# AechPro/rlgym-ppo

Measured on AMD Instinct MI355X. Metric: ppo_update_samples_per_sec, higher is better.
Workload: dtype f32; 1 GPU; configs[1]: 4096 agents x 128 steps = 524,288-sample buffer, obs 107 f32, 90 discrete actions, 256x3 policy + critic; batch 524,288, minibatch 65,536

## Files before the change

### rlgym_ppo_amd/csrc/api.hip

```cpp
#include "build_id.h"
#include <math.h>
#include <stdarg.h>
#include <string.h>

#include "common.hpp"

namespace rlppo {

static thread_local char g_err[512] = "";

void set_error(const char *fmt, ...) {
    va_list ap;
    va_start(ap, fmt);
    vsnprintf(g_err, sizeof(g_err), fmt, ap);
    va_end(ap);
}

static int64_t padded_width(int64_t d) {
    const int64_t p16 = round_up(d, 16), p64 = round_up(d, 64);
    return (p64 - p16) * 10 >= p64 ? p16 : p64;
}
static int64_t padded_out(int64_t d) {
    if (d <= 32) return 32;
    if (d <= 64) return 64;
// ... 39 lines not shown

struct X3Layout {
    int64_t fwd[RLPPO_MAX_LAYERS], dx[RLPPO_MAX_LAYERS], total;
};
static void x3_layout(const NetLayout &net, X3Layout *o) {
    int64_t off = 0;
    const int last = net.n_layers - 1;
    for (int l = 0; l < net.n_layers; ++l) {
        const LayerLayout &L = net.L[l];
        o->fwd[l] = o->dx[l] = -1;
        if (l >= 1 && l < last && nt_split_ok(L.pout, L.pin)) {
            o->fwd[l] = off;
            off += (int64_t)3 * L.pout * L.pin;
        }
        if (l >= 1 && !(l == last && gemv_head_ok(L.out, L.pin)) && nt_split_ok(L.pin, L.pout)) {
            o->dx[l] = off;
            off += (int64_t)3 * L.pin * L.pout;
        }
    }
    o->total = off;
}

static int g_fold_vhead = 1;

struct RowSource {
    const float *x;
    int64_t ld;
    const unsigned *rowtab = nullptr;
    int64_t src_rows = 0;
};

static int forward(hipStream_t st, const NetLayout &net, const float *packed, const RowSource &in, int64_t n, int out_tanh,
                   float *const *acts, int bf16_operands = 0, unsigned long long *const *bits = nullptr, bool *have_bits = nullptr,
                   bool *head_folded = nullptr, const unsigned short *x3 = nullptr, bool head_prezeroed = false) {
    X3Layout xl;
    if (x3) x3_layout(net, &xl);
    if (have_bits)
        for (int l = 0; l < net.n_layers; ++l) have_bits[l] = false;
    const float *x = in.x;
    int64_t ldx = in.ld;
    const int hl = net.n_layers - 1;
    bool fold = head_folded && g_fold_vhead && hl >= 1 && !out_tanh && !bf16_operands && bits && bits[hl - 1] &&
                gemv_head_ok(net.L[hl].out, net.L[hl].pin) && net.L[hl - 1].pout / 128 <= 2;
    if (x3 && hl >= 1 && xl.fwd[hl - 1] >= 0) fold = false;
    if (head_folded) *head_folded = false;
    for (int l = 0; l < net.n_layers; ++l) {
        const LayerLayout &L = net.L[l];
        const bool last = l == net.n_layers - 1;
        const int epi = last ? (out_tanh ? EPI_BIAS_TANH : EPI_BIAS) : EPI_BIAS_RELU;
        int rc;
        if (last && head_folded && *head_folded) break;
        if (last && !out_tanh && gemv_head_ok(L.out, L.pin))
            rc = launch_gemv_fwd(st, x, ldx, packed + L.off_w, packed + L.off_b, acts[l], L.pout, n, L.pin, L.pout);
        else {
            rc = -1;
            if (!last && bits && bits[l] && x3 && xl.fwd[l] >= 0) {
                rc = launch_gemm_nt_split(st, x, ldx, x3 + xl.fwd[l], packed + L.off_b, acts[l], L.pout, n, L.pout, L.pin, 0, bits[l]);
                if (rc == 0) have_bits[l] = true;
            } else if (!last && bits && bits[l] && !bf16_operands) {
                NtDot dots[2];
                const bool fold_here = fold && l == hl - 1;
                if (fold_here) {
                    if (!head_prezeroed) RLPPO_HIP(hipMemsetAsync(acts[hl], 0, (size_t)n * sizeof(float), st));
                    dots[0].w = packed + net.L[hl].off_w;
                    dots[0].b = packed + net.L[hl].off_b;
                    dots[0].out = acts[hl];
                }
                rc = launch_gemm_nt_bits(st, x, ldx, packed + L.off_w, L.pin, packed + L.off_b, acts[l], L.pout, n, L.pout, L.pin,
                                         EPI_BIAS_RELU, bits[l], l == 0 ? in.rowtab : nullptr, in.src_rows, nullptr, fold_here ? dots : nullptr);
                if (rc == 0) have_bits[l] = true;
                if (fold_here) *head_folded = rc == 0;
            }
            if (l == 0 && in.rowtab && rc != 0) {
                if (rc == -1) set_error("forward: the gathered first layer needs the bitmask form");
                return rc == -1 ? RLPPO_ERR_ARG : rc;
            }
            if (rc == -1)
                rc = launch_gemm_nt(st, x, ldx, packed + L.off_w, L.pin, packed + L.off_b, nullptr, 0, acts[l], L.pout, n, L.pout,
                                    L.pin, epi, bf16_operands);
        }
        if (rc) return rc;
        x = acts[l];
        ldx = L.pout;
    }
// ... 67 lines not shown
        ldx = L.pout;
    }
    return 0;
}

static size_t forward_ws_floats(const NetLayout &net, int64_t n) { return (size_t)2 * (size_t)n * (size_t)max_pout(net); }

static int forward_pingpong(hipStream_t st, const NetLayout &net, const float *packed, const float *obs, int64_t ld_obs,
                            int64_t n, int out_tanh, void *ws, size_t ws_bytes, float *final_out, const float **out,
                            int64_t *ld_out, int bf16_operands) {
    if (ws_bytes < forward_ws_floats(net, n) * sizeof(float)) {
        set_error("forward: workspace %zu < %zu bytes", ws_bytes, forward_ws_floats(net, n) * sizeof(float));
        return RLPPO_ERR_WORKSPACE;
    }
    RLPPO_CHECK_ARG(ld_obs >= net.L[0].pin && ld_obs % 4 == 0, "forward: ld_obs=%ld must be >= %d (zero padded rows)",
                    (long)ld_obs, net.L[0].pin);
    float *b0 = reinterpret_cast<float *>(ws);
    float *b1 = b0 + (size_t)n * max_pout(net);
    float *acts[RLPPO_MAX_LAYERS];
    for (int l = 0; l < net.n_layers; ++l) acts[l] = (l & 1) ? b1 : b0;
    if (final_out) acts[net.n_layers - 1] = final_out;
    int rc = forward(st, net, packed, RowSource{obs, ld_obs}, n, out_tanh, acts, bf16_operands);
    if (rc) return rc;
    *out = acts[net.n_layers - 1];
    *ld_out = net.L[net.n_layers - 1].pout;
    return 0;
}

}

using namespace rlppo;

static int g_fused_act = 1;
static std::atomic<long long> g_cnt_fused_act{0}, g_cnt_act_chain{0}, g_cnt_paired_pass{0}, g_cnt_gather_fused_pass{0}, g_cnt_pass{0}, g_cnt_group_dw{0};
constexpr int64_t FUSED_ACT_MAX_ROWS = 8192;

struct ActCtx {
    int bf16 = 0;
    unsigned *done = nullptr;
    unsigned done_value = 0;
    unsigned *noise_ctl = nullptr;
};
static int act_ctx(const rlppo_act_opts *o, ActCtx *c, bool late_noise = false) {
    c->bf16 = get_infer_bf16();
    if (!o) return 0;
    RLPPO_CHECK_ARG(o->precision == RLPPO_PRECISION_DEFAULT || o->precision == RLPPO_PRECISION_FP32 || o->precision == RLPPO_PRECISION_BF16,
                    "act options: inference precision %d (0 = process default, 1 = fp32, 2 = bf16 operands)", o->precision);
    if (o->precision != RLPPO_PRECISION_DEFAULT) c->bf16 = o->precision == RLPPO_PRECISION_BF16;
    c->done = o->done_words;
    c->done_value = o->done_value;
    c->noise_ctl = o->noise_ctl;
    RLPPO_CHECK_ARG(!o->noise_ctl || late_noise, "act options: noise_ctl is an option of rlppo_discrete_step");
    RLPPO_CHECK_ARG(!o->noise_ctl || (o->done_words && !(o->done_value & 0x80000000u)),
                    "act options: noise_ctl needs done_words (a kernel that gives up on the noise reports it there) and done_value < 2^31");
    return 0;
}
static int act_done(hipStream_t st, const ActCtx &c, int64_t n) {
    return c.done ? launch_signal_words(st, c.done, (int)rlppo_act_done_words(n), c.done_value) : 0;
}

extern "C" {

int rlppo_abi_version(void) { return RLPPO_ABI_VERSION; }
const char *rlppo_build_id(void) { return RLPPO_BUILD_ID; }
const char *rlppo_last_error(void) { return g_err; }

int64_t rlppo_padded_width(int64_t d) { return padded_width(d); }
// ... 656 lines not shown
    hipStream_t st, side;
    DwList *defer;
};

static LossCfg loss_cfg(const rlppo_minibatch_args &a) {
    LossCfg c;
    c.clip = a.clip_range;
    c.clip_lo = (float)(1.0 - (double)a.clip_range);
    c.clip_hi = (float)(1.0 + (double)a.clip_range);
    c.ent_coef = a.ent_coef;
    c.mb_ratio = a.mb_ratio;
    c.inv_mb = 1.0f / (float)a.mb;
    c.var_m = a.var_m;
    c.var_b = a.var_b;
    c.adv_norm = a.adv_norm;
    c.vclip = a.value_clip;
    c.kl_slots = a.kl_slots;
    c.stop_word = a.stop_word;
    return c;
}

static int policy_loss(hipStream_t st, const Pass &p) {
    const rlppo_minibatch_args &a = *p.a;
    const int last = p.pol.n_layers - 1;
    const LayerLayout &L = p.pol.L[last];
    const WsPlan &w = p.w;
    if (a.head == RLPPO_HEAD_DISCRETE)
        return launch_discrete_loss(st, w.pol.act[last], L.pout, L.out, w.g_act, w.g_old, w.g_adv, p.mb, p.cfg, a.stats);
    if (a.head == RLPPO_HEAD_GAUSSIAN)
        return launch_gaussian_loss(st, w.pol.act[last], L.pout, L.out / 2, w.g_act, w.g_old, w.g_adv, p.mb, p.cfg, a.stats);
    return launch_multidiscrete_loss(st, w.pol.act[last], L.pout, w.g_act, w.g_old, w.g_adv, p.mb, p.cfg, a.stats);
}

static int gather(const Pass &p) {
    const rlppo_minibatch_args &a = *p.a;
    const WsPlan &w = p.w;
    const int width = p.pol.L[0].pin;
    float *const vout = w.val.act[p.val.n_layers - 1];
    if (p.prec == 1) {
        auto lean0 = [](const NetLayout &n) {
            return n.n_layers > 1 && nt_b16_ok(n.L[0].pout, n.L[0].pin, true) && tn_b16_ok(n.L[0].pout, n.L[0].pin);
        };
        const int rc = launch_gather_rows_round(p.st, a.states, a.ld_states, a.idx, lean0(p.pol) && lean0(p.val) ? nullptr : w.states,
                                                w.states_b, width, p.mb, p.ring_base, p.ring_cap);
        if (rc) return rc;
    } else if (!p.rows.rowtab) {
        GatherMeta gm;
        gm.actions = a.actions; gm.old_logp = a.old_logp; gm.adv = a.advantages; gm.targets = a.targets;
        gm.g_old = w.g_old; gm.g_adv = w.g_adv; gm.g_tgt = w.g_tgt; gm.g_act = w.g_act;
        gm.zero_n = vout;
        gm.act_dim = a.act_dim;
        return launch_gather_rows(p.st, a.states, a.ld_states, a.idx, w.states, width, p.mb, p.ring_base, p.ring_cap, &gm);
    }
    return launch_gather_meta(p.st, a.idx, a.actions, a.act_dim, a.old_logp, a.advantages, a.targets, w.g_act, w.g_old, w.g_adv, w.g_tgt,
                              p.mb, p.ring_base, p.ring_cap, p.rows.rowtab ? w.rowtab : nullptr, vout);
}

static int paired_pass(const Pass &p, SlotBank &bk, int slot) {
    const rlppo_minibatch_args &a = *p.a;
    const NetLayout &pol = p.pol, &val = p.val;
    const WsPlan &w = p.w;
    const int64_t mb = p.mb;
    const hipStream_t st = p.st, hs = p.side;
    const int H = pol.n_layers - 1;
    int rc;
    const LayerLayout &Lvh = val.L[H];
// ... 8 lines not shown
        alt.A = xv;
        alt.B = p.val_w + Lv.off_w;
        alt.bias = p.val_w + Lv.off_b;
        alt.C = w.val.act[l];
        alt.bits = w.val.bits[l];
        NtDot dots[2];
        const bool fold_here = fold_v && l == H - 1;
        if (fold_here) {
            dots[1].w = p.val_w + Lvh.off_w;
            dots[1].out = vout;
            dots[1].b = p.val_w + Lvh.off_b;
        }
        rc = launch_gemm_nt_bits(st, xp, ldx, p.pol_w + Lp.off_w, Lp.pin, p.pol_w + Lp.off_b, w.pol.act[l], Lp.pout, mb, Lp.pout, Lp.pin,
                                 EPI_BIAS_RELU, w.pol.bits[l], l == 0 ? p.rows.rowtab : nullptr, p.rows.src_rows, &alt,
                                 fold_here ? dots : nullptr);
        if (rc) {
            if (rc == -1) set_error("paired pass: a hidden layer does not have the bitmask form");
            return rc == -1 ? RLPPO_ERR_ARG : rc;
        }
        xp = w.pol.act[l];
        xv = w.val.act[l];
        ldx = Lp.pout;
    }
    if (hs != st) {
        rc = order_after(hs, st, bk.ev_fork[slot]);
        if (rc) return rc;
    }
    if (!fold_v) {
        rc = head_forward(hs, val, p.val_w, xv, ldx, mb, 0, vout);
        if (rc) return rc;
    }
    rc = launch_value_loss(hs, vout, ldv, w.g_tgt, w.g_adv, mb, p.cfg, a.stats);
    if (rc) return rc;
    const bool ordered = g_head_order && hs != st;
    if (!ordered) {
        rc = head_backward(hs, val, p.val_w, vout, xv, mb, w.val.dx[H - 1], a.val_grad, w.val.tn, w.val.bits[H - 1], ldv, p.defer);
        if (rc) return rc;
    }
    rc = head_forward(st, pol, p.pol_w, xp, ldx, mb, a.head == RLPPO_HEAD_GAUSSIAN, pout);
    if (rc) return rc;
    rc = policy_loss(st, p);
    if (rc) return rc;
    if (ordered) {
        rc = order_after(hs, st, bk.ev_mid[slot]);
        if (rc) return rc;
        rc = head_backward(hs, val, p.val_w, vout, xv, mb, w.val.dx[H - 1], a.val_grad, w.val.tn, w.val.bits[H - 1], ldv, p.defer);
        if (rc) return rc;
    }
    rc = head_backward(st, pol, p.pol_w, pout, xp, mb, w.pol.dx[H - 1], a.pol_grad, w.pol.tn, w.pol.bits[H - 1], 0, p.defer);
    if (rc) return rc;
    if (hs != st) {
        rc = order_after(st, hs, bk.ev_join[slot]);
        if (rc) return rc;
    }
    for (int l = H - 1; l >= 0; --l) {
        const LayerLayout &Lp = pol.L[l], &Lv = val.L[l];
        const RowSource Xp = l > 0 ? RowSource{w.pol.act[l - 1], pol.L[l - 1].pout} : p.rows;
        const RowSource Xv = l > 0 ? RowSource{w.val.act[l - 1], val.L[l - 1].pout} : p.rows;
        if (p.defer) {
            p.defer->add(Lp, w.pol.dx[l], Xp, a.pol_grad);
            p.defer->add(Lv, w.val.dx[l], Xv, a.val_grad);
        } else {
            TnPair pr;
            pr.dY = w.val.dx[l];
            pr.X = Xv.x;
            pr.dW = a.val_grad + Lv.off_flat_w;
            pr.db = a.val_grad + Lv.off_flat_b;
            pr.ws = w.val.tn;
            rc = launch_gemm_tn(st, w.pol.dx[l], Lp.pout, Lp.pout, Xp.x, Xp.ld, Lp.pin, a.pol_grad + Lp.off_flat_w, a.pol_grad + Lp.off_flat_b,
                                Lp.out, Lp.in, mb, w.pol.tn, tn_layer_floats(pol, l, mb, 0), Xp.rowtab, Xp.src_rows, &pr);
            if (rc) return rc;
        }
        if (l == 0) break;
        NtAlt alt;
        alt.A = w.val.dx[l];
        alt.B = p.val_w + Lv.off_wt;
        alt.C = w.val.dx[l - 1];
        alt.bits = w.val.bits[l - 1];
        rc = launch_gemm_nt_bits(st, w.pol.dx[l], Lp.pout, p.pol_w + Lp.off_wt, Lp.pout, nullptr, w.pol.dx[l - 1], Lp.pin, mb, Lp.pin,
                                 Lp.pout, EPI_MASK, w.pol.bits[l - 1], nullptr, 0, &alt);
        if (rc) return rc == -1 ? RLPPO_ERR_ARG : rc;
    }
    return 0;
}

static int two_chain_pass(const Pass &p) {
    const rlppo_minibatch_args &a = *p.a;
    const NetLayout &pol = p.pol, &val = p.val;
    const WsPlan &w = p.w;
    const int64_t mb = p.mb;
    const bool b16 = p.prec == 1;
    const unsigned short *pol_wb16 = reinterpret_cast<const unsigned short *>(a.pol_wb16);
    const unsigned short *val_wb16 = reinterpret_cast<const unsigned short *>(a.val_wb16);
    const unsigned short *pol_x3 = p.prec == 2 ? pol_wb16 : nullptr, *val_x3 = p.prec == 2 ? val_wb16 : nullptr;
    bool phave[RLPPO_MAX_LAYERS] = {}, vhave[RLPPO_MAX_LAYERS] = {};
    bool pf32[RLPPO_MAX_LAYERS] = {}, vf32[RLPPO_MAX_LAYERS] = {};
    bool v_folded = false;
    int rc;
    if (b16) {
        rc = forward_b16(p.side, val, p.val_w, val_wb16, p.rows.x, w.states_b, p.rows.ld, mb, 0, w.val.act, w.val.actb, w.val.bits, vhave,
                         vf32);
        if (rc) return rc;
        rc = forward_b16(p.st, pol, p.pol_w, pol_wb16, p.rows.x, w.states_b, p.rows.ld, mb, a.head == RLPPO_HEAD_GAUSSIAN, w.pol.act,
                         w.pol.actb, w.pol.bits, phave, pf32);
    } else {
        rc = forward(p.side, val, p.val_w, p.rows, mb, 0, w.val.act, 0, w.val.bits, vhave, &v_folded, val_x3, true);
        if (rc) return rc;
        rc = forward(p.st, pol, p.pol_w, p.rows, mb, a.head == RLPPO_HEAD_GAUSSIAN, w.pol.act, 0, w.pol.bits, phave, nullptr, pol_x3);
    }
    if (rc) return rc;
    const int64_t ldv = v_folded ? 1 : val.L[val.n_layers - 1].pout;
    rc = launch_value_loss(p.side, w.val.act[val.n_layers - 1], ldv, w.g_tgt, w.g_adv, mb, p.cfg, a.stats);
    if (rc) return rc;
    rc = policy_loss(p.st, p);
    if (rc) return rc;
    if (b16) {
        rc = backward_b16(p.side, val, p.val_w, val_wb16, p.rows.x, w.states_b, p.rows.ld, mb, w.val.act, w.val.actb, w.val.dx, w.val.dxb,
                          a.val_grad, w.val.tn, tn_ws_floats(val, mb, p.prec), w.val.bits, vhave, vf32);
        if (rc) return rc;
        return backward_b16(p.st, pol, p.pol_w, pol_wb16, p.rows.x, w.states_b, p.rows.ld, mb, w.pol.act, w.pol.actb, w.pol.dx, w.pol.dxb,
                            a.pol_grad, w.pol.tn, tn_ws_floats(pol, mb, p.prec), w.pol.bits, phave, pf32);
    }
    rc = backward(p.side, val, p.val_w, p.rows, mb, w.val.act, w.val.dx, a.val_grad, w.val.tn, w.val.bits, vhave, v_folded, val_x3, p.defer);
    if (rc) return rc;
    return backward(p.st, pol, p.pol_w, p.rows, mb, w.pol.act, w.pol.dx, a.pol_grad, w.pol.tn, w.pol.bits, phave, false, pol_x3, p.defer);
}

int rlppo_ppo_minibatch(void *stream, const rlppo_minibatch_args *a) {
    RLPPO_CHECK_ARG(a != nullptr, "ppo_minibatch: null args");
    Pass p;
    p.a = a;
    int rc = make_layout(a->pol_dims, a->pol_layers, &p.pol);
    if (rc) return rc;
    rc = make_layout(a->val_dims, a->val_layers, &p.val);
    if (rc) return rc;
    const NetLayout &pol = p.pol, &val = p.val;
    const int64_t mb = p.mb = a->mb;
    if (mb == 0) return 0;
    rc = resolve_precision(a->precision, &p.prec);
    if (rc) return rc;
    RLPPO_CHECK_ARG(mb > 0 && a->pol_packed && a->val_packed && a->pol_grad && a->val_grad && a->states && a->actions &&
                        a->old_logp && a->targets && a->advantages && a->idx && a->stats && a->workspace,
                    "ppo_minibatch: null pointer");
    RLPPO_CHECK_ARG(val.L[val.n_layers - 1].out == 1, "ppo_minibatch: critic must have one output");
    RLPPO_CHECK_ARG(a->value_clip >= 0.f && a->value_clip < INFINITY, "ppo_minibatch: value_clip=%g", (double)a->value_clip);
    RLPPO_CHECK_ARG(pol.L[0].in == val.L[0].in, "ppo_minibatch: policy and critic observe different sizes");
    RLPPO_CHECK_ARG(a->ld_states >= pol.L[0].pin && a->ld_states % 4 == 0, "ppo_minibatch: ld_states=%ld < %d",
// ... 232 lines not shown
    g_update_bf16 = mode;
    ++g_selection_epoch;
    return 0;
}
int rlppo_get_update_precision(void) { return g_update_bf16; }
int rlppo_set_inference_precision(int32_t mode) {
    RLPPO_CHECK_ARG(mode == 0 || mode == 1, "set_inference_precision: mode %d (0 = fp32, 1 = bf16 operands)", mode);
    set_infer_bf16(mode);
    ++g_selection_epoch;
    return 0;
}
int rlppo_dbg_set(int32_t key, int32_t value) {
    ++g_selection_epoch;
    switch (key) {
        case 1: set_gae_algo(value); return 0;
        case 4: g_two_streams = value; return 0;
        case 21: set_gae_spin_limit(value); return 0;
        case 22: set_gae_oversubscribe(value); return 0;
        case 34: set_fused_spin_limit(value); return 0;
        case 35: set_fused_test_hold(value); return 0;
        case 36: set_split_persistent(value); return 0;
        case 23: set_b16_wide_tiles(value); return 0;
        case 24: set_exp_fast_transform(value); return 0;
        case 26: g_fused_gather = value; return 0;
        case 27: g_fused_act = value; return 0;
        case 29: g_paired = value; return 0;
        case 31: g_head_order = value; return 0;
        case 32: g_fold_vhead = value; return 0;
        case 33: set_pair_interleave(value); return 0;
        case 37: g_group_dw = value; return 0;
        case 38: set_tn_group_budget(value); return 0;
        case 40: set_nt_skinny(value); return 0;
        case 41: g_window_mode = value; return 0;
        default: break;
    }
    set_error("dbg_set: unknown key %d", key);
    return RLPPO_ERR_ARG;
}
int64_t rlppo_selection_epoch(void) { return g_selection_epoch; }
const int64_t *rlppo_selection_epoch_ptr(void) { return &g_selection_epoch; }
int64_t rlppo_dbg_counter(int32_t key) {
    switch (key) {
        case 0: return g_cnt_fused_act;
        case 1: return g_cnt_act_chain;
        case 2: return g_cnt_pass;
        case 3: return g_cnt_paired_pass;
        case 4: return g_cnt_gather_fused_pass;
        case 5: return g_cnt_group_dw;
        default: return -1;
    }
}
size_t rlppo_dbg_gemm_nt_bits_bytes(int64_t M, int32_t N) { return nt_bits_floats(M, N) * sizeof(float); }
int rlppo_dbg_gemm_nt_bits(void *stream, const float *A, int64_t lda, const float *B, int64_t ldb, const float *bias, float *C,
                           int64_t ldc, int64_t M, int32_t N, int32_t K, int32_t epilogue, void *bits) {
    const int rc = launch_gemm_nt_bits((hipStream_t)stream, A, lda, B, ldb, bias, C, ldc, M, N, K, epilogue,
                                       reinterpret_cast<unsigned long long *>(bits));
    if (rc == -1) {
        set_error("dbg_gemm_nt_bits: the bitmask form does not apply to this call");
        return RLPPO_ERR_ARG;
    }
    return rc;
}
int rlppo_dbg_gemm_nt(void *stream, const float *A, int64_t lda, const float *B, int64_t ldb, const float *bias,
                      const float *mask_src, int64_t ld_mask, float *C, int64_t ldc, int64_t M, int32_t N, int32_t K,
                      int32_t epilogue) {
    return launch_gemm_nt((hipStream_t)stream, A, lda, B, ldb, bias, mask_src, ld_mask, C, ldc, M, N, K, epilogue);
}
int rlppo_dbg_gemm_nt_b16(void *stream, const void *A, int64_t lda, const void *W, int64_t ldw, const float *bias, float *C,
                          int64_t ldc, void *Cb, int64_t ldcb, int64_t M, int32_t N, int32_t K, int32_t epilogue, int32_t hidden,
                          void *bits) {
    return launch_gemm_nt_b16((hipStream_t)stream, reinterpret_cast<const unsigned short *>(A), lda,
                              reinterpret_cast<const unsigned short *>(W), ldw, bias, C, ldc, reinterpret_cast<unsigned short *>(Cb),
                              ldcb, M, N, K, epilogue, hidden, reinterpret_cast<unsigned long long *>(bits));
}
int rlppo_dbg_gemm_tn_b16(void *stream, const void *dY, int64_t ldy, const void *X, int64_t ldx, float *dW, float *db, int32_t pout,
                          int32_t pin, int32_t out, int32_t in, int64_t M, void *ws, size_t ws_bytes) {
    return launch_gemm_tn_b16((hipStream_t)stream, reinterpret_cast<const unsigned short *>(dY), ldy,
                              reinterpret_cast<const unsigned short *>(X), ldx, dW, db, pout, pin, out, in, M, (float *)ws,
                              ws_bytes / sizeof(float));
}
size_t rlppo_dbg_thin_head_workspace_bytes(int32_t out, int32_t kp, int64_t M) { return thin_dw_ws_floats(out, kp, M) * sizeof(float); }
// ... 42 lines not shown
```

### rlgym_ppo_amd/csrc/common.hpp

```cpp
#pragma once
#include <hip/hip_runtime.h>
#include <stdint.h>
#include <stdio.h>

#include <atomic>

#include "../../include/rlppo.h"

namespace rlppo {

void set_error(const char *fmt, ...);

#define RLPPO_CHECK_ARG(cond, ...)                \
    do {                                          \
        if (!(cond)) {                            \
            rlppo::set_error(__VA_ARGS__);        \
            return RLPPO_ERR_ARG;                 \
        }                                         \
    } while (0)

#define RLPPO_HIP(expr)                                                                         \
    do {                                                                                        \
        hipError_t e_ = (expr);                                                                 \
        if (e_ != hipSuccess) {                                                                 \
// ... 134 lines not shown
int launch_thin_dw_b16(hipStream_t st, const float *dy, int64_t ldy, const unsigned short *xb, int64_t ldx, float *dw, float *db,
                       int out, int in, int kp, int64_t n, float *ws, size_t ws_floats);
int launch_gemv_dx(hipStream_t st, const float *dy, int64_t ldy, const float *w, const float *mask, int64_t ldm, float *dx, int64_t ldc, int kp, int64_t n);
int launch_gemv_dx_bits(hipStream_t st, const float *dy, int64_t ldy, const float *w, const unsigned long long *bits, float *dx,
                        int64_t ldc, int kp, int64_t n);
int launch_gemv_dw(hipStream_t st, const float *dy, int64_t ldy, const float *x, int64_t ldx, float *dw, float *db, int in, int kp, int64_t n,
                   float *ws = nullptr, size_t ws_floats = 0);

struct LossCfg {
    float clip, clip_lo, clip_hi, ent_coef, mb_ratio, inv_mb;
    float var_m, var_b;
    const float *adv_norm = nullptr;
    float vclip = 0.f;
    double *kl_slots = nullptr;
    const unsigned *stop_word = nullptr;
};
__host__ __device__ __forceinline__ int64_t ring_row(int64_t i, int64_t base, int64_t cap) {
    const int64_t r = i + base;
    return r >= cap ? r - cap : r;
}
int launch_discrete_sample_logits(hipStream_t, const float *, int64_t, int64_t, int, const float *, int64_t *, float *, float *);
int launch_discrete_probs(hipStream_t st, const float *logits, int64_t ld, int64_t n, int A, int clamp, float *probs,
                          int64_t ld_p, int64_t *flat_argmax);
int launch_categorical_select(hipStream_t, const float *, int64_t, int64_t, int, const float *, int64_t *, float *);
int launch_gaussian_sample(hipStream_t, const float *, int64_t, int64_t, int, const float *, float, float, float *, float *,
                           unsigned *done_words = nullptr, unsigned done_value = 0);
int launch_multidiscrete_sample(hipStream_t, const float *, int64_t, int64_t, const float *, int64_t *, float *,
                                unsigned *done_words = nullptr, unsigned done_value = 0);
int launch_value_loss(hipStream_t st, float *vout, int64_t ldv, const float *targets, const float *adv, int64_t mb, const LossCfg &cfg,
                      double *stats);
int64_t kl_slots_doubles(int64_t mb);
constexpr int64_t DISCRETE_LOSS_MAX_LD = 64 * 32;
int launch_discrete_loss(hipStream_t, float *, int64_t, int, const float *, const float *, const float *, int64_t, const LossCfg &, double *);
int launch_gaussian_loss(hipStream_t, float *, int64_t, int, const float *, const float *, const float *, int64_t, const LossCfg &, double *);
int launch_multidiscrete_loss(hipStream_t, float *, int64_t, const float *, const float *, const float *, int64_t, const LossCfg &, double *);

struct FusedActIO {
    const float *rows = nullptr;
    int64_t ld_rows = 0;
    const void *raw = nullptr;
    int raw_is_f64 = 0, standardize = 0;
    int64_t ld_raw = 0;
    float mean0 = 0.f, std0 = 1.f;
    const float *mean_v = nullptr, *std_v = nullptr;
    float *rows_out = nullptr;
    int64_t ld_rows_out = 0;
    const float *noise = nullptr;
    int64_t *actions = nullptr;
    float *actions_f32 = nullptr;
    float *logp = nullptr, *probs_out = nullptr;
    unsigned *done_words = nullptr;
    unsigned done_value = 0;
    unsigned *noise_ctl = nullptr;
};
bool fused_act_ok(const NetLayout &net);
}
void host_window_register(void *base, size_t bytes, unsigned *hdp_flush);
void host_window_unregister(void *base);
namespace rlppo {
int launch_discrete_act_fused(hipStream_t st, const NetLayout &net, const float *packed, const FusedActIO &io, int64_t n);

size_t gae_workspace_bytes(int64_t n);
void set_gae_algo(int algo);
void set_gae_spin_limit(int v);
void set_gae_oversubscribe(int v);
void set_fused_spin_limit(int v);
// ... 40 lines not shown
```

### rlgym_ppo_amd/csrc/heads.hip

```cpp
#include "common.hpp"

namespace rlppo {

constexpr float PROB_MIN = 1e-11f;

__device__ __forceinline__ float wave_max(float v) {
#pragma unroll
    for (int o = 32; o > 0; o >>= 1) v = fmaxf(v, __shfl_xor(v, o));
    return v;
}
__device__ __forceinline__ float wave_sum(float v) {
#pragma unroll
    for (int o = 32; o > 0; o >>= 1) v += __shfl_xor(v, o);
    return v;
}

template <int EPL>
__device__ __forceinline__ void row_softmax(const float *__restrict__ z, int A, int lane, float (&p)[EPL],
                                            float (&pc)[EPL]) {
    float mx = -INFINITY;
#pragma unroll
    for (int e = 0; e < EPL; ++e) {
        const int c = lane + 64 * e;
        p[e] = c < A ? z[c] : -INFINITY;
        mx = fmaxf(mx, p[e]);
    }
    mx = wave_max(mx);
    float s = 0.f;
#pragma unroll
    for (int e = 0; e < EPL; ++e) {
        const int c = lane + 64 * e;
        p[e] = c < A ? expf(p[e] - mx) : 0.f;
        s += p[e];
// ... 257 lines not shown
        for (int e = 0; e < EPL; ++e) {
            const int c = lane + 64 * e;
            if (c < ld) z[c] = c < A ? p[e] * (gp[e] - dot) : 0.f;
        }
        if (lane == 0) {
            st[RLPPO_STAT_ENTROPY] += ent * cfg.inv_mb;
            st[RLPPO_STAT_KL] += ((ratio - 1.f) - lr) * cfg.inv_mb;
            st[RLPPO_STAT_CLIPFRAC] += (fabsf(ratio - 1.f) > cfg.clip ? 1.f : 0.f) * cfg.inv_mb;
            st[RLPPO_STAT_PLOSS] += -smin * cfg.inv_mb;
        }
    }
    block_stats_add(stats, st, true, cfg, cfg.kl_slots);
}

template <int CTRL>
__device__ __forceinline__ float dpp_mov(float v) {
    return __builtin_bit_cast(float, __builtin_amdgcn_update_dpp(0, __builtin_bit_cast(int, v), CTRL, 0xF, 0xF, true));
}
__device__ __forceinline__ float row16_sum(float v) {
    v += dpp_mov<0xB1>(v);
    v += dpp_mov<0x4E>(v);
    v += dpp_mov<0x141>(v);
    v += dpp_mov<0x140>(v);
    return v;
}
__device__ __forceinline__ float row16_max(float v) {
    v = fmaxf(v, dpp_mov<0xB1>(v));
    v = fmaxf(v, dpp_mov<0x4E>(v));
    v = fmaxf(v, dpp_mov<0x141>(v));
    v = fmaxf(v, dpp_mov<0x140>(v));
    return v;
}

__global__ __launch_bounds__(256) void discrete_loss16_kernel(float *__restrict__ logits, int64_t ld, int A,
                                                               const float *__restrict__ actions,
                                                               const float *__restrict__ old_logp,
                                                               const float *__restrict__ advantages, int64_t mb,
                                                               LossCfg cfg, double *__restrict__ stats) {
    typedef float f32x4 __attribute__((ext_vector_type(4)));
    const int l16 = threadIdx.x & 15, grp = threadIdx.x >> 4;
    const int c0 = l16 * 8;
    const bool in_row = c0 < ld;
    float st[5] = {0.f, 0.f, 0.f, 0.f, 0.f};
    for (int64_t base = (int64_t)blockIdx.x * 16; base < mb; base += (int64_t)gridDim.x * 16) {
        const bool live = base + grp < mb;
        const int64_t row = live ? base + grp : mb - 1;
        float *z = logits + row * ld + c0;
        float p[8], pc[8], lp[8];
        if (in_row) {
            const f32x4 z0 = *reinterpret_cast<const f32x4 *>(z), z1 = *reinterpret_cast<const f32x4 *>(z + 4);
#pragma unroll
            for (int e = 0; e < 4; ++e) {
                p[e] = z0[e];
                p[4 + e] = z1[e];
            }
        }
        const float old = old_logp[row], adv = surrogate_adv(advantages[row], cfg);
        const int a = (int)actions[row];
        float mx = -INFINITY;
#pragma unroll
        for (int e = 0; e < 8; ++e) {
            if (!(in_row && c0 + e < A)) p[e] = -INFINITY;
            mx = fmaxf(mx, p[e]);
        }
        mx = row16_max(mx);
        float s = 0.f;
#pragma unroll
        for (int e = 0; e < 8; ++e) {
            p[e] = (c0 + e < A) ? expf(p[e] - mx) : 0.f;
            s += p[e];
        }
        s = row16_sum(s);
        float ent = 0.f, lpa = 0.f, pca = 0.f;
#pragma unroll
        for (int e = 0; e < 8; ++e) {
            const int c = c0 + e;
            p[e] = p[e] / s;
            pc[e] = fminf(fmaxf(p[e], PROB_MIN), 1.0f);
            lp[e] = c < A ? logf(pc[e]) : 0.f;
            if (c < A) ent -= lp[e] * pc[e];
            if (c == a) {
                lpa = lp[e];
                pca = pc[e];
            }
        }
        ent = row16_sum(ent);
        lpa = row16_sum(lpa);
        pca = row16_sum(pca);
        const float lr = lpa - old;
        const float ratio = expf(lr);
        float smin;
        const float w = surrogate_weight(ratio, adv, cfg, smin);
        const float g_logp = cfg.mb_ratio * (-(adv * w * ratio) * cfg.inv_mb);
        const float g_ent = cfg.mb_ratio * (cfg.ent_coef * cfg.inv_mb);
        float gp[8];
        float dot = 0.f;
#pragma unroll
        for (int e = 0; e < 8; ++e) {
            const int c = c0 + e;
            float g = 0.f;
            if (c < A) {
                g = g_ent * (lp[e] + 1.f);
                if (c == a) g += g_logp / pca;
                if (!(p[e] >= PROB_MIN)) g = 0.f;
            }
            gp[e] = g;
            dot += g * p[e];
        }
        dot = row16_sum(dot);
        if (live && in_row) {
            f32x4 o0, o1;
#pragma unroll
            for (int e = 0; e < 4; ++e) {
                o0[e] = (c0 + e < A) ? p[e] * (gp[e] - dot) : 0.f;
                o1[e] = (c0 + 4 + e < A) ? p[4 + e] * (gp[4 + e] - dot) : 0.f;
            }
            *reinterpret_cast<f32x4 *>(z) = o0;
            *reinterpret_cast<f32x4 *>(z + 4) = o1;
        }
        if (live && l16 == 0) {
            st[RLPPO_STAT_ENTROPY] += ent * cfg.inv_mb;
            st[RLPPO_STAT_KL] += ((ratio - 1.f) - lr) * cfg.inv_mb;
            st[RLPPO_STAT_CLIPFRAC] += (fabsf(ratio - 1.f) > cfg.clip ? 1.f : 0.f) * cfg.inv_mb;
            st[RLPPO_STAT_PLOSS] += -smin * cfg.inv_mb;
        }
    }
    block_stats_add(stats, st, true, cfg, cfg.kl_slots);
}

__global__ __launch_bounds__(256) void value_loss_kernel(float *__restrict__ vout, int64_t ldv, const float *__restrict__ targets,
                                                         const float *__restrict__ advantages, int64_t mb, LossCfg cfg,
                                                         double *__restrict__ stats) {
    float st[5] = {0.f, 0.f, 0.f, 0.f, 0.f};
    for (int64_t row = (int64_t)blockIdx.x * 256 + threadIdx.x; row < mb; row += (int64_t)gridDim.x * 256)
        st[RLPPO_STAT_VLOSS] += value_row(vout + row * ldv, targets[row], cfg.vclip > 0.f ? advantages[row] : 0.f, cfg) * cfg.inv_mb;
    block_stats_add(stats, st, true, cfg);
}

int launch_value_loss(hipStream_t st, float *vout, int64_t ldv, const float *targets, const float *adv, int64_t mb, const LossCfg &cfg,
                      double *stats) {
    if (mb <= 0) return 0;
    RLPPO_CHECK_ARG(!(cfg.vclip > 0.f) || adv, "value loss: clipping needs the advantages");
    dim3 grid((unsigned)(cdiv(mb, 256) < 1024 ? cdiv(mb, 256) : 1024));
    hipLaunchKernelGGL(value_loss_kernel, grid, dim3(256), 0, st, vout, ldv, targets, adv, mb, cfg, stats);
    RLPPO_LAUNCH_CHECK();
    return 0;
}

int64_t kl_slots_doubles(int64_t mb) {
    const int64_t g = cdiv(mb > 0 ? mb : 1, 256);
    return 2 + (g > 2048 ? g : 2048);
}

int launch_discrete_loss(hipStream_t st, float *logits, int64_t ld, int A, const float *actions, const float *old_logp, const float *adv,
                         int64_t mb, const LossCfg &cfg, double *stats) {
    if (mb <= 0) return 0;
    dim3 grid((unsigned)(cdiv(mb, 4) < 2048 ? cdiv(mb, 4) : 2048)), block(256);
    RLPPO_CHECK_ARG(ld <= DISCRETE_LOSS_MAX_LD, "discrete head: padded width %ld too large", (long)ld);
    if (ld <= 128) {
        dim3 grid16((unsigned)(cdiv(mb, 16) < 2048 ? cdiv(mb, 16) : 2048));
        hipLaunchKernelGGL(discrete_loss16_kernel, grid16, block, 0, st, logits, ld, A, actions, old_logp, adv, mb, cfg, stats);
    } else if (ld <= 512)
        hipLaunchKernelGGL((discrete_loss_kernel<8>), grid, block, 0, st, logits, ld, A, actions, old_logp, adv, mb, cfg, stats);
    else
        hipLaunchKernelGGL((discrete_loss_kernel<32>), grid, block, 0, st, logits, ld, A, actions, old_logp, adv, mb, cfg, stats);
    RLPPO_LAUNCH_CHECK();
    return 0;
}

constexpr int FLOAT_SUM_K = 32;

__device__ __forceinline__ float gauss_logpdf(float x, float mean, float sd) {
    const float msq = mean * mean, ssq = sd * sd, xsq = x * x;
    const float t1 = -(msq / (2.f * ssq));
    const float t2 = (mean * x) / ssq;
    const float t3 = -(xsq / (2.f * ssq));
    const float t4 = logf(1.f / sqrtf((float)(2.0 * 3.14159265358979323846) * ssq));
    return t1 + t2 + t3 + t4;
}

__device__ __forceinline__ void block_done_words(unsigned *done_words, unsigned done_value, int64_t n) {
    if (!done_words) return;
    __builtin_amdgcn_fence(__ATOMIC_RELEASE, "");
    __syncthreads();
    const int64_t w = (int64_t)blockIdx.x * 16 + threadIdx.x;
    if (threadIdx.x < 16 && w < (n + 15) / 16) __hip_atomic_store(done_words + w, done_value, __ATOMIC_RELEASE, __HIP_MEMORY_SCOPE_SYSTEM);
}

__global__ __launch_bounds__(256) void gaussian_sample_kernel(const float *__restrict__ y, int64_t ld, int64_t n, int k,
                                                               const float *__restrict__ eps, float var_m, float var_b,
                                                               float *__restrict__ actions, float *__restrict__ logp,
                                                               unsigned *done_words, unsigned done_value) {
    const int64_t row = (int64_t)blockIdx.x * blockDim.x + threadIdx.x;
    if (row < n) {
        const float *yr = y + row * ld;
        float lp = 0.f;
        double lpd = 0.0;
        for (int j = 0; j < k; ++j) {
// ... 206 lines not shown
```

Baseline: 64.10 million samples/s.

## Fuse discrete policy head GEMM with softmax PPO loss and gradient

Adds a kernel that computes the policy head logits with MFMA tiles, parks each tile in LDS, and runs the discrete softmax/PPO loss and logit-gradient directly on it. Per-row stat terms go to a buffer and a small replay kernel reduces them in the same grouping as before. The separate head forward GEMM and loss kernel, along with the global round trip of the logits, are dropped for the fp32 discrete path without KL slots. The cost is an extra terms buffer and a second small launch.

```diff
diff --git a/rlgym_ppo_amd/csrc/api.hip b/rlgym_ppo_amd/csrc/api.hip
--- a/rlgym_ppo_amd/csrc/api.hip
+++ b/rlgym_ppo_amd/csrc/api.hip
@@ -95,7 +95,7 @@
 
 static int forward(hipStream_t st, const NetLayout &net, const float *packed, const RowSource &in, int64_t n, int out_tanh,
                    float *const *acts, int bf16_operands = 0, unsigned long long *const *bits = nullptr, bool *have_bits = nullptr,
-                   bool *head_folded = nullptr, const unsigned short *x3 = nullptr, bool head_prezeroed = false) {
+                   bool *head_folded = nullptr, const unsigned short *x3 = nullptr, bool head_prezeroed = false, bool skip_head = false) {
     X3Layout xl;
     if (x3) x3_layout(net, &xl);
     if (have_bits)
@@ -112,7 +112,7 @@
         const bool last = l == net.n_layers - 1;
         const int epi = last ? (out_tanh ? EPI_BIAS_TANH : EPI_BIAS) : EPI_BIAS_RELU;
         int rc;
-        if (last && head_folded && *head_folded) break;
+        if (last && ((head_folded && *head_folded) || skip_head)) break;
         if (last && !out_tanh && gemv_head_ok(L.out, L.pin))
             rc = launch_gemv_fwd(st, x, ldx, packed + L.off_w, packed + L.off_b, acts[l], L.pout, n, L.pin, L.pout);
         else {
@@ -246,7 +246,7 @@
 using namespace rlppo;
 
 static int g_fused_act = 1;
-static std::atomic<long long> g_cnt_fused_act{0}, g_cnt_act_chain{0}, g_cnt_paired_pass{0}, g_cnt_gather_fused_pass{0}, g_cnt_pass{0}, g_cnt_group_dw{0};
+static std::atomic<long long> g_cnt_fused_act{0}, g_cnt_act_chain{0}, g_cnt_paired_pass{0}, g_cnt_gather_fused_pass{0}, g_cnt_pass{0}, g_cnt_group_dw{0}, g_cnt_head_chain{0};
 constexpr int64_t FUSED_ACT_MAX_ROWS = 8192;
 
 struct ActCtx {
@@ -969,6 +969,24 @@
     return launch_multidiscrete_loss(st, w.pol.act[last], L.pout, w.g_act, w.g_old, w.g_adv, p.mb, p.cfg, a.stats);
 }
 
+static int g_head_chain = 1;
+static bool head_chain_ok(const Pass &p) {
+    const int H = p.pol.n_layers - 1;
+    if (!g_head_chain || p.prec != 0 || p.a->head != RLPPO_HEAD_DISCRETE || p.cfg.kl_slots || H < 1) return false;
+    const LayerLayout &L = p.pol.L[H];
+    return discrete_head_chain_ok(L.pout, L.pin, p.pol.L[H - 1].pout);
+}
+static int policy_head_chain(hipStream_t st, const Pass &p) {
+    const rlppo_minibatch_args &a = *p.a;
+    const int H = p.pol.n_layers - 1;
+    const LayerLayout &L = p.pol.L[H];
+    const WsPlan &w = p.w;
+    float *terms = reinterpret_cast<float *>((reinterpret_cast<uintptr_t>(w.g_act + p.mb) + 15) & ~(uintptr_t)15);
+    ++g_cnt_head_chain;
+    return launch_discrete_head_chain(st, w.pol.act[H - 1], p.pol.L[H - 1].pout, p.pol_w + L.off_w, p.pol_w + L.off_b, L.pin, w.pol.act[H],
+                                      L.pout, L.out, w.g_act, w.g_old, w.g_adv, p.mb, p.cfg, a.stats, terms);
+}
+
 static int gather(const Pass &p) {
     const rlppo_minibatch_args &a = *p.a;
     const WsPlan &w = p.w;
@@ -1043,14 +1061,18 @@
     }
     rc = launch_value_loss(hs, vout, ldv, w.g_tgt, w.g_adv, mb, p.cfg, a.stats);
     if (rc) return rc;
-    const bool ordered = g_head_order && hs != st;
+    const bool chain = head_chain_ok(p);
+    const bool ordered = g_head_order && hs != st && (!chain || g_head_order == 2);
     if (!ordered) {
         rc = head_backward(hs, val, p.val_w, vout, xv, mb, w.val.dx[H - 1], a.val_grad, w.val.tn, w.val.bits[H - 1], ldv, p.defer);
         if (rc) return rc;
     }
-    rc = head_forward(st, pol, p.pol_w, xp, ldx, mb, a.head == RLPPO_HEAD_GAUSSIAN, pout);
-    if (rc) return rc;
-    rc = policy_loss(st, p);
+    if (chain) {
+        rc = policy_head_chain(st, p);
+    } else {
+        rc = head_forward(st, pol, p.pol_w, xp, ldx, mb, a.head == RLPPO_HEAD_GAUSSIAN, pout);
+        if (rc == 0) rc = policy_loss(st, p);
+    }
     if (rc) return rc;
     if (ordered) {
         rc = order_after(hs, st, bk.ev_mid[slot]);
@@ -1107,6 +1129,7 @@
     bool phave[RLPPO_MAX_LAYERS] = {}, vhave[RLPPO_MAX_LAYERS] = {};
     bool pf32[RLPPO_MAX_LAYERS] = {}, vf32[RLPPO_MAX_LAYERS] = {};
     bool v_folded = false;
+    const bool chain = head_chain_ok(p);
     int rc;
     if (b16) {
         rc = forward_b16(p.side, val, p.val_w, val_wb16, p.rows.x, w.states_b, p.rows.ld, mb, 0, w.val.act, w.val.actb, w.val.bits, vhave,
@@ -1117,13 +1140,14 @@
     } else {
         rc = forward(p.side, val, p.val_w, p.rows, mb, 0, w.val.act, 0, w.val.bits, vhave, &v_folded, val_x3, true);
         if (rc) return rc;
-        rc = forward(p.st, pol, p.pol_w, p.rows, mb, a.head == RLPPO_HEAD_GAUSSIAN, w.pol.act, 0, w.pol.bits, phave, nullptr, pol_x3);
+        rc = forward(p.st, pol, p.pol_w, p.rows, mb, a.head == RLPPO_HEAD_GAUSSIAN, w.pol.act, 0, w.pol.bits, phave, nullptr, pol_x3, false,
+                     chain);
     }
     if (rc) return rc;
     const int64_t ldv = v_folded ? 1 : val.L[val.n_layers - 1].pout;
     rc = launch_value_loss(p.side, w.val.act[val.n_layers - 1], ldv, w.g_tgt, w.g_adv, mb, p.cfg, a.stats);
     if (rc) return rc;
-    rc = policy_loss(p.st, p);
+    rc = chain ? policy_head_chain(p.st, p) : policy_loss(p.st, p);
     if (rc) return rc;
     if (b16) {
         rc = backward_b16(p.side, val, p.val_w, val_wb16, p.rows.x, w.states_b, p.rows.ld, mb, w.val.act, w.val.actb, w.val.dx, w.val.dxb,
@@ -1422,6 +1446,7 @@
         case 38: set_tn_group_budget(value); return 0;
         case 40: set_nt_skinny(value); return 0;
         case 41: g_window_mode = value; return 0;
+        case 42: g_head_chain = value; return 0;
         default: break;
     }
     set_error("dbg_set: unknown key %d", key);
@@ -1437,6 +1462,7 @@
         case 3: return g_cnt_paired_pass;
         case 4: return g_cnt_gather_fused_pass;
         case 5: return g_cnt_group_dw;
+        case 6: return g_cnt_head_chain;
         default: return -1;
     }
 }
diff --git a/rlgym_ppo_amd/csrc/common.hpp b/rlgym_ppo_amd/csrc/common.hpp
--- a/rlgym_ppo_amd/csrc/common.hpp
+++ b/rlgym_ppo_amd/csrc/common.hpp
@@ -190,6 +190,10 @@
 int64_t kl_slots_doubles(int64_t mb);
 constexpr int64_t DISCRETE_LOSS_MAX_LD = 64 * 32;
 int launch_discrete_loss(hipStream_t, float *, int64_t, int, const float *, const float *, const float *, int64_t, const LossCfg &, double *);
+bool discrete_head_chain_ok(int ld, int K, int64_t ldx);
+int launch_discrete_head_chain(hipStream_t st, const float *X, int64_t ldx, const float *W, const float *bias, int K, float *dZ, int ld, int A,
+                               const float *actions, const float *old_logp, const float *adv, int64_t mb, const LossCfg &cfg, double *stats,
+                               float *terms);
 int launch_gaussian_loss(hipStream_t, float *, int64_t, int, const float *, const float *, const float *, int64_t, const LossCfg &, double *);
 int launch_multidiscrete_loss(hipStream_t, float *, int64_t, const float *, const float *, const float *, int64_t, const LossCfg &, double *);
 
diff --git a/rlgym_ppo_amd/csrc/heads.hip b/rlgym_ppo_amd/csrc/heads.hip
--- a/rlgym_ppo_amd/csrc/heads.hip
+++ b/rlgym_ppo_amd/csrc/heads.hip
@@ -1,4 +1,4 @@
-#include "common.hpp"
+#include "gemm_detail.hpp"
 
 namespace rlppo {
 
@@ -322,12 +322,77 @@
     return v;
 }
 
+__device__ __forceinline__ void discrete_row16(float (&p)[8], bool in_row, int c0, int A, float old, float adv, int a, const LossCfg &cfg,
+                                               f32x4 &o0, f32x4 &o1, float (&t)[5]) {
+    float pc[8], lp[8];
+    float mx = -INFINITY;
+#pragma unroll
+    for (int e = 0; e < 8; ++e) {
+        if (!(in_row && c0 + e < A)) p[e] = -INFINITY;
+        mx = fmaxf(mx, p[e]);
+    }
+    mx = row16_max(mx);
+    float s = 0.f;
+#pragma unroll
+    for (int e = 0; e < 8; ++e) {
+        p[e] = (c0 + e < A) ? expf(p[e] - mx) : 0.f;
+        s += p[e];
+    }
+    s = row16_sum(s);
+    float ent = 0.f, lpa = 0.f, pca = 0.f;
+#pragma unroll
+    for (int e = 0; e < 8; ++e) {
+        const int c = c0 + e;
+        p[e] = p[e] / s;
+        pc[e] = fminf(fmaxf(p[e], PROB_MIN), 1.0f);
+        lp[e] = c < A ? logf(pc[e]) : 0.f;
+        if (c < A) ent -= lp[e] * pc[e];
+        if (c == a) {
+            lpa = lp[e];
+            pca = pc[e];
+        }
+    }
+    ent = row16_sum(ent);
+    lpa = row16_sum(lpa);
+    pca = row16_sum(pca);
+    const float lr = lpa - old;
+    const float ratio = expf(lr);
+    float smin;
+    const float w = surrogate_weight(ratio, adv, cfg, smin);
+    const float g_logp = cfg.mb_ratio * (-(adv * w * ratio) * cfg.inv_mb);
+    const float g_ent = cfg.mb_ratio * (cfg.ent_coef * cfg.inv_mb);
+    float gp[8];
+    float dot = 0.f;
+#pragma unroll
+    for (int e = 0; e < 8; ++e) {
+        const int c = c0 + e;
+        float g = 0.f;
+        if (c < A) {
+            g = g_ent * (lp[e] + 1.f);
+            if (c == a) g += g_logp / pca;
+            if (!(p[e] >= PROB_MIN)) g = 0.f;
+        }
+        gp[e] = g;
+        dot += g * p[e];
+    }
+    dot = row16_sum(dot);
+#pragma unroll
+    for (int e = 0; e < 4; ++e) {
+        o0[e] = (c0 + e < A) ? p[e] * (gp[e] - dot) : 0.f;
+        o1[e] = (c0 + 4 + e < A) ? p[4 + e] * (gp[4 + e] - dot) : 0.f;
+    }
+    t[RLPPO_STAT_ENTROPY] = ent * cfg.inv_mb;
+    t[RLPPO_STAT_KL] = ((ratio - 1.f) - lr) * cfg.inv_mb;
+    t[RLPPO_STAT_VLOSS] = 0.f;
+    t[RLPPO_STAT_CLIPFRAC] = (fabsf(ratio - 1.f) > cfg.clip ? 1.f : 0.f) * cfg.inv_mb;
+    t[RLPPO_STAT_PLOSS] = -smin * cfg.inv_mb;
+}
+
 __global__ __launch_bounds__(256) void discrete_loss16_kernel(float *__restrict__ logits, int64_t ld, int A,
                                                                const float *__restrict__ actions,
                                                                const float *__restrict__ old_logp,
                                                                const float *__restrict__ advantages, int64_t mb,
                                                                LossCfg cfg, double *__restrict__ stats) {
-    typedef float f32x4 __attribute__((ext_vector_type(4)));
     const int l16 = threadIdx.x & 15, grp = threadIdx.x >> 4;
     const int c0 = l16 * 8;
     const bool in_row = c0 < ld;
@@ -336,7 +401,7 @@
         const bool live = base + grp < mb;
         const int64_t row = live ? base + grp : mb - 1;
         float *z = logits + row * ld + c0;
-        float p[8], pc[8], lp[8];
+        float p[8];
         if (in_row) {
             const f32x4 z0 = *reinterpret_cast<const f32x4 *>(z), z1 = *reinterpret_cast<const f32x4 *>(z + 4);
 #pragma unroll
@@ -347,72 +412,18 @@
         }
         const float old = old_logp[row], adv = surrogate_adv(advantages[row], cfg);
         const int a = (int)actions[row];
-        float mx = -INFINITY;
-#pragma unroll
-        for (int e = 0; e < 8; ++e) {
-            if (!(in_row && c0 + e < A)) p[e] = -INFINITY;
-            mx = fmaxf(mx, p[e]);
-        }
-        mx = row16_max(mx);
-        float s = 0.f;
-#pragma unroll
-        for (int e = 0; e < 8; ++e) {
-            p[e] = (c0 + e < A) ? expf(p[e] - mx) : 0.f;
-            s += p[e];
-        }
-        s = row16_sum(s);
-        float ent = 0.f, lpa = 0.f, pca = 0.f;
-#pragma unroll
-        for (int e = 0; e < 8; ++e) {
-            const int c = c0 + e;
-            p[e] = p[e] / s;
-            pc[e] = fminf(fmaxf(p[e], PROB_MIN), 1.0f);
-            lp[e] = c < A ? logf(pc[e]) : 0.f;
-            if (c < A) ent -= lp[e] * pc[e];
-            if (c == a) {
-                lpa = lp[e];
-                pca = pc[e];
-            }
-        }
-        ent = row16_sum(ent);
-        lpa = row16_sum(lpa);
-        pca = row16_sum(pca);
-        const float lr = lpa - old;
-        const float ratio = expf(lr);
-        float smin;
-        const float w = surrogate_weight(ratio, adv, cfg, smin);
-        const float g_logp = cfg.mb_ratio * (-(adv * w * ratio) * cfg.inv_mb);
-        const float g_ent = cfg.mb_ratio * (cfg.ent_coef * cfg.inv_mb);
-        float gp[8];
-        float dot = 0.f;
-#pragma unroll
-        for (int e = 0; e < 8; ++e) {
-            const int c = c0 + e;
-            float g = 0.f;
-            if (c < A) {
-                g = g_ent * (lp[e] + 1.f);
-                if (c == a) g += g_logp / pca;
-                if (!(p[e] >= PROB_MIN)) g = 0.f;
-            }
-            gp[e] = g;
-            dot += g * p[e];
-        }
-        dot = row16_sum(dot);
+        f32x4 o0, o1;
+        float t[5];
+        discrete_row16(p, in_row, c0, A, old, adv, a, cfg, o0, o1, t);
         if (live && in_row) {
-            f32x4 o0, o1;
-#pragma unroll
-            for (int e = 0; e < 4; ++e) {
-                o0[e] = (c0 + e < A) ? p[e] * (gp[e] - dot) : 0.f;
-                o1[e] = (c0 + 4 + e < A) ? p[4 + e] * (gp[4 + e] - dot) : 0.f;
-            }
             *reinterpret_cast<f32x4 *>(z) = o0;
             *reinterpret_cast<f32x4 *>(z + 4) = o1;
         }
         if (live && l16 == 0) {
-            st[RLPPO_STAT_ENTROPY] += ent * cfg.inv_mb;
-            st[RLPPO_STAT_KL] += ((ratio - 1.f) - lr) * cfg.inv_mb;
-            st[RLPPO_STAT_CLIPFRAC] += (fabsf(ratio - 1.f) > cfg.clip ? 1.f : 0.f) * cfg.inv_mb;
-            st[RLPPO_STAT_PLOSS] += -smin * cfg.inv_mb;
+            st[RLPPO_STAT_ENTROPY] += t[RLPPO_STAT_ENTROPY];
+            st[RLPPO_STAT_KL] += t[RLPPO_STAT_KL];
+            st[RLPPO_STAT_CLIPFRAC] += t[RLPPO_STAT_CLIPFRAC];
+            st[RLPPO_STAT_PLOSS] += t[RLPPO_STAT_PLOSS];
         }
     }
     block_stats_add(stats, st, true, cfg, cfg.kl_slots);
@@ -454,6 +465,183 @@
         hipLaunchKernelGGL((discrete_loss_kernel<8>), grid, block, 0, st, logits, ld, A, actions, old_logp, adv, mb, cfg, stats);
     else
         hipLaunchKernelGGL((discrete_loss_kernel<32>), grid, block, 0, st, logits, ld, A, actions, old_logp, adv, mb, cfg, stats);
+    RLPPO_LAUNCH_CHECK();
+    return 0;
+}
+
+template <int NB>
+__global__ __launch_bounds__(256, 4) void discrete_head_chain_kernel(const float *__restrict__ X, unsigned ldx_b, const float *__restrict__ W,
+                                                                     unsigned ldw_b, const float *__restrict__ bias, int K,
+                                                                     float *__restrict__ dZ, int A, const float *__restrict__ actions,
+                                                                     const float *__restrict__ old_logp,
+                                                                     const float *__restrict__ advantages, int64_t mb, LossCfg cfg,
+                                                                     f32x4 *__restrict__ terms) {
+    constexpr int BKT = 16;
+    constexpr int BN = NB * 16;
+    constexpr int CPR = BKT / 4;
+    constexpr int RPW = 64 / CPR;
+    constexpr int RPP = 4 * RPW;
+    constexpr int A_IT = SBM / RPP, B_IT = BN / RPP;
+    constexpr int B_REM = BN % RPP;
+    static_assert(B_REM % RPW == 0, "the ragged staging pass must be whole wave instructions");
+    constexpr int PLD = BN + 4;
+    constexpr int STAGE_F = 2 * SBM * BKT + 2 * BN * BKT, PARK_F = 4 * 16 * PLD;
+    __shared__ __attribute__((aligned(16))) float lds[STAGE_F > PARK_F ? STAGE_F : PARK_F];
+    float *As = lds;
+    float *Bs = lds + 2 * SBM * BKT;
+
+    const int tid = threadIdx.x;
+    const int lane = tid & 63, wave = tid >> 6;
+    const int wave_u = __builtin_amdgcn_readfirstlane(wave);
+    const int r16 = lane & 15, q = lane >> 4;
+    const int64_t m0 = (int64_t)blockIdx.x * SBM;
+    const int rows_here = (int)((mb - m0) < SBM ? (mb - m0) : SBM);
+
+    const __amdgpu_buffer_rsrc_t a_rs = make_rsrc(reinterpret_cast<const char *>(X) + m0 * ldx_b, (unsigned)(rows_here - 1) * ldx_b + (unsigned)K * 4);
+    const __amdgpu_buffer_rsrc_t b_rs = make_rsrc(W, (unsigned)(BN - 1) * ldw_b + (unsigned)K * 4);
+    const int row_p = wave * RPW + lane / CPR, pch = lane % CPR;
+    const int lch = pch ^ ((0 - (row_p >> 2)) & 3);
+    const unsigned a_off = (unsigned)row_p * ldx_b + lch * 16;
+    const unsigned b_off = (unsigned)row_p * ldw_b + lch * 16;
+    const unsigned a_step = (unsigned)RPP * ldx_b, b_step = (unsigned)RPP * ldw_b;
+
+    f32x4 acc[2][NB];
+    {
+        const __amdgpu_buffer_rsrc_t bias_rs = make_rsrc(bias, BN * 4);
+#pragma unroll
+        for (int j = 0; j < NB; ++j) {
+            acc[0][j] = ldb(bias_rs, (unsigned)(q * 16), j * 64);
+            acc[1][j] = acc[0][j];
+        }
+    }
+    auto issue_tile = [&](int buf, unsigned kb) {
+        float *Ad = As + buf * SBM * BKT + wave_u * RPW * BKT;
+        float *Bd = Bs + buf * BN * BKT + wave_u * RPW * BKT;
+#pragma unroll
+        for (int i = 0; i < A_IT; ++i) __builtin_amdgcn_raw_ptr_buffer_load_lds(a_rs, Ad + i * RPP * BKT, 16, a_off, kb + i * a_step, 0, 0);
+#pragma unroll
+        for (int i = 0; i < B_IT; ++i) __builtin_amdgcn_raw_ptr_buffer_load_lds(b_rs, Bd + i * RPP * BKT, 16, b_off, kb + i * b_step, 0, 0);
+        if (B_REM != 0 && wave_u * RPW < B_REM)
+            __builtin_amdgcn_raw_ptr_buffer_load_lds(b_rs, Bd + B_IT * RPP * BKT, 16, b_off, kb + B_IT * b_step, 0, 0);
+    };
+    const int nk = K / BKT;
+    issue_tile(0, 0);
+    asm volatile("s_waitcnt vmcnt(0)" ::: "memory");
+    __syncthreads();
+    for (int kt = 0; kt < nk; ++kt) {
+        const int cur = kt & 1;
+        if ((kt + 1) < nk) issue_tile(cur ^ 1, (unsigned)(kt + 1) * (BKT * 4));
+        const float *Ac = As + cur * SBM * BKT + (wave * 32) * BKT;
+        const float *Bc = Bs + cur * BN * BKT;
+        f32x4 fa[2], fb[NB];
+#pragma unroll
+        for (int i = 0; i < 2; ++i) fa[i] = *reinterpret_cast<const f32x4 *>(&Ac[dswz<BKT>(i * 16 + r16, q)]);
+#pragma unroll
+        for (int j = 0; j < NB; ++j) fb[j] = *reinterpret_cast<const f32x4 *>(&Bc[dswz<BKT>(j * 16 + r16, q)]);
+#pragma unroll
+        for (int s = 0; s < 4; ++s)
+#pragma unroll
+            for (int i = 0; i < 2; ++i)
+#pragma unroll
+                for (int j = 0; j < NB; ++j) acc[i][j] = MFMA16(fb[j][s], fa[i][s], acc[i][j]);
+        __builtin_amdgcn_sched_barrier(0);
+        asm volatile("s_waitcnt vmcnt(0)" ::: "memory");
+        __syncthreads();
+    }
+
+    float *const park = lds + wave_u * 16 * PLD;
+    const int l16 = lane & 15, grp = lane >> 4, c0 = l16 * 8;
+    const bool in_row = c0 < BN;
+#pragma unroll
+    for (int i = 0; i < 2; ++i) {
+        if (i) asm volatile("s_waitcnt lgkmcnt(0)" ::: "memory");
+#pragma unroll
+        for (int j = 0; j < NB; ++j) *reinterpret_cast<f32x4 *>(park + r16 * PLD + 16 * j + 4 * q) = acc[i][j];
+#pragma unroll
+        for (int t = 0; t < 4; ++t) {
+            const int rl = 4 * t + grp;
+            const int64_t row_u = m0 + wave * 32 + 16 * i + rl;
+            const bool live = row_u < mb;
+            const int64_t row = live ? row_u : mb - 1;
+            float p[8];
+            if (in_row) {
+                const f32x4 z0 = *reinterpret_cast<const f32x4 *>(park + rl * PLD + c0), z1 = *reinterpret_cast<const f32x4 *>(park + rl * PLD + c0 + 4);
+#pragma unroll
+                for (int e = 0; e < 4; ++e) {
+                    p[e] = z0[e];
+                    p[4 + e] = z1[e];
+                }
+            }
+            const float old = old_logp[row], adv = surrogate_adv(advantages[row], cfg);
+            const int a = (int)actions[row];
+            f32x4 o0, o1;
+            float tr[5];
+            discrete_row16(p, in_row, c0, A, old, adv, a, cfg, o0, o1, tr);
+            if (live && in_row) {
+                float *z = dZ + row * BN + c0;
+                *reinterpret_cast<f32x4 *>(z) = o0;
+                *reinterpret_cast<f32x4 *>(z + 4) = o1;
+            }
+            if (live && l16 == 0)
+                terms[row] = f32x4{tr[RLPPO_STAT_ENTROPY], tr[RLPPO_STAT_KL], tr[RLPPO_STAT_CLIPFRAC], tr[RLPPO_STAT_PLOSS]};
+        }
+    }
+}
+
+__global__ __launch_bounds__(256) void discrete_stats_replay_kernel(const f32x4 *__restrict__ terms, int64_t mb, int G, LossCfg cfg,
+                                                                    double *__restrict__ stats) {
+    const int lane = threadIdx.x & 63, grp = threadIdx.x & 15;
+    const int b = (int)blockIdx.x * 16 + (int)(threadIdx.x >> 4);
+    float s[5] = {0.f, 0.f, 0.f, 0.f, 0.f};
+    if (b < G) {
+#pragma unroll 4
+        for (int64_t row = (int64_t)b * 16 + grp; row < mb; row += (int64_t)G * 16) {
+            const f32x4 t = terms[row];
+            s[RLPPO_STAT_ENTROPY] += t[0];
+            s[RLPPO_STAT_KL] += t[1];
+            s[RLPPO_STAT_CLIPFRAC] += t[2];
+            s[RLPPO_STAT_PLOSS] += t[3];
+        }
+    }
+    double d[5];
+#pragma unroll
+    for (int k = 0; k < 5; ++k) {
+        float x = s[k];
+        x += __shfl_xor(x, 2);
+        x += __shfl_xor(x, 1);
+        const int g0 = lane & ~15;
+        d[k] = (double)__shfl(x, g0) + (double)__shfl(x, g0 + 4) + (double)__shfl(x, g0 + 8) + (double)__shfl(x, g0 + 12);
+    }
+    if (b < G && grp == 0 && !(cfg.stop_word && *cfg.stop_word)) {
+#pragma unroll
+        for (int k = 0; k < 5; ++k) atomicAdd(stats + k, d[k]);
+    }
+}
+
+bool discrete_head_chain_ok(int ld, int K, int64_t ldx) {
+    const int64_t lim = (int64_t)1 << 31;
+    return (ld == 32 || ld == 64 || ld == 96 || ld == 128) && K > 0 && K % 16 == 0 && ldx >= K && ldx % 4 == 0 && 129 * ldx * 4 < lim &&
+           129 * (int64_t)K * 4 < lim;
+}
+int launch_discrete_head_chain(hipStream_t st, const float *X, int64_t ldx, const float *W, const float *bias, int K, float *dZ, int ld, int A,
+                               const float *actions, const float *old_logp, const float *adv, int64_t mb, const LossCfg &cfg, double *stats,
+                               float *terms) {
+    if (mb <= 0) return 0;
+    RLPPO_CHECK_ARG(discrete_head_chain_ok(ld, K, ldx) && A <= ld && (reinterpret_cast<uintptr_t>(terms) & 15) == 0,
+                    "discrete head chain: unsupported shape (ld %d, K %d, ldx %ld)", ld, K, (long)ldx);
+    f32x4 *t4 = reinterpret_cast<f32x4 *>(terms);
+    const dim3 grid((unsigned)cdiv(mb, SBM)), block(256);
+    const unsigned lx = (unsigned)(ldx * 4), lw = (unsigned)K * 4;
+#define HC(NB)                                                                                                                         \
+    case NB * 16:                                                                                                                      \
+        hipLaunchKernelGGL((discrete_head_chain_kernel<NB>), grid, block, 0, st, X, lx, W, lw, bias, K, dZ, A, actions, old_logp, adv, \
+                           mb, cfg, t4);                                                                                               \
+        break;
+    switch (ld) { HC(2) HC(4) HC(6) HC(8) }
+#undef HC
+    RLPPO_LAUNCH_CHECK();
+    const int G = (int)(cdiv(mb, 16) < 2048 ? cdiv(mb, 16) : 2048);
+    hipLaunchKernelGGL(discrete_stats_replay_kernel, dim3((unsigned)cdiv(G, 16)), block, 0, st, t4, mb, G, cfg, stats);
     RLPPO_LAUNCH_CHECK();
     return 0;
 }
```

Result: no change. 64.37 million samples/s (median of 6 runs) (+0.4%).
